# drwangxian/viterbi_spl

Hardware: AMD Instinct MI355X
Metric: Viterbi Mframes/s at S=361 T=30k; achieved HBM GB/s vs peak (higher is better)
Workload: dtype f32

## Files before the change

### viterbi_spl_amd/csrc/banded.hip

```cpp
#include "device_common.hpp"

namespace vit {

template <int W, int NWT, bool DW, bool DBG, int NXT, typename ET>
__global__ void __launch_bounds__((NWT + (DW ? 3 : 2)) * 64) banded_forward_kernel(FwdArgs a) {
    extern __shared__ __align__(16) unsigned char smem[];
    constexpr int NP = NWT * 64;
    constexpr int EPL = NWT;
    const int S = a.S, SP = a.SP, T = a.T, SD = a.SD;
    constexpr int DC = NP + 16;
    float* dls = reinterpret_cast<float*>(smem);
    float* dl = dls + 4;
    float* Pv = dls + 4 * DC;
    float* Sv = Pv + NP + 1;
    float* Dv = Sv + NP + 1;
    VI* tot = reinterpret_cast<VI*>(Dv + kMaxDenseRows);

    const int tid = threadIdx.x;
    const int lane = tid & 63;
    const int wv = __builtin_amdgcn_readfirstlane(tid >> 6);
    const int song = blockIdx.x;
    const int Tb = song_length(a.lengths, song, T);
    const ET* __restrict__ E = reinterpret_cast<const ET*>(a.logE) + (size_t)song * T * S;
    float* __restrict__ hist = a.hist + (size_t)song * T * SD;
// ... 85 lines not shown
        unsigned long long v;
        asm volatile("s_memtime %0\n\ts_waitcnt lgkmcnt(0)" : "=s"(v)::"memory");
        return v;
    };
    auto frame = [&](const int t, float& e_slot) {
        float m = -INFINITY;
        const bool prof = (dbg & 256) != 0;
        const unsigned long long s0 = prof ? stamp() : 0ull;
        if (is_target) {
            float m0 = -INFINITY, m1 = -INFINITY, m2 = -INFINITY, m3 = -INFINITY;
            float xd[NXL > 0 ? NXL : 1];
#pragma unroll
            for (int k = 0; k < NXL; ++k) xd[k] = (!GEN || k < nx) ? dl[xcol[k]] : -INFINITY;
            if (!(dbg & 1)) {
                const f32x4* __restrict__ win = reinterpret_cast<const f32x4*>(dl + (lo & 3) * DC + (lo & ~3));
#pragma unroll
                for (int w = 0; w + 7 < W; w += 8) {
                    const f32x4 da = win[w / 4], db = win[w / 4 + 1];
                    const f32x2 c0_ = f32x2{da.x, da.y} + f32x2{aw[w + 0], aw[w + 1]};
                    const f32x2 c1_ = f32x2{da.z, da.w} + f32x2{aw[w + 2], aw[w + 3]};
                    const f32x2 c2_ = f32x2{db.x, db.y} + f32x2{aw[w + 4], aw[w + 5]};
                    const f32x2 c3_ = f32x2{db.z, db.w} + f32x2{aw[w + 6], aw[w + 7]};
                    m0 = fmaxf(fmaxf(m0, c0_.x), c0_.y);
                    m1 = fmaxf(fmaxf(m1, c1_.x), c1_.y);
                    m2 = fmaxf(fmaxf(m2, c2_.x), c2_.y);
                    m3 = fmaxf(fmaxf(m3, c3_.x), c3_.y);
                }
            }
#pragma unroll
            for (int k = 0; k < NXL; ++k) m1 = fmaxf(m1, xd[k] + xa[k]);
            m = fmaxf(fmaxf(m0, m1), fmaxf(m2, m3));
        } else if (!(dbg & 2)) {
            float d[EPL];
#pragma unroll
            for (int e = 0; e < EPL; ++e) d[e] = dl[i0 + e];
            if (role == 0) {
                float p[EPL];
                float run = -INFINITY;
#pragma unroll
                for (int e = 0; e < EPL; ++e) {
                    run = fmaxf(run, smask[e] ? -INFINITY : d[e]);
                    p[e] = run;
                }
                const float inc = wave_scan_max(run);
                const float ex = wave_shift_up(inc, -INFINITY);
#pragma unroll
                for (int e = 0; e < EPL; ++e) Pv[i0 + e + 1] = fmaxf(ex, p[e]);
                if (lane == 63 && !(dbg & 8)) hist[(size_t)(t - 1) * SD + S] = inc;
            } else {
                if (role == 1) {
                    float p[EPL];
                    float run = -INFINITY;
#pragma unroll
                    for (int e = EPL - 1; e >= 0; --e) {
                        run = fmaxf(run, smask[e] ? -INFINITY : d[e]);
                        p[e] = run;
                    }
                    const float ex = wave_shift_up(wave_scan_max(run), -INFINITY);
#pragma unroll
                    for (int e = 0; e < EPL; ++e) Sv[i0 + e] = fmaxf(ex, p[e]);
                }
                if (GEN && role == kDenseRole) {
#pragma unroll
                    for (int dr = 0; dr < kMaxDenseRows; ++dr) {
                        if (dr < nd) {
                            float dm = -INFINITY;
#pragma unroll
                            for (int e = 0; e < EPL; ++e) dm = fmaxf(dm, d[e] + dA[dr][e]);
                            dm = wave_max_all(dm);
                            if (lane == 0) Dv[dr] = dm;
                        }
                    }
                }
            }
        }
        const unsigned long long s1 = prof ? stamp() : 0ull;
        __syncthreads();
        const unsigned long long s2 = prof ? stamp() : 0ull;

        if (is_target && !(dbg & 4)) {
            m = fmaxf(m, fmaxf(Pv[lo], Sv[lo + W]) + cj);
            if (GEN) {
                const float dres = Dv[kind >= 0 ? kind : 0];
                if (kind >= 0) m = dres;
            }
            {
                const float dn = tvalid ? m + e_slot : -INFINITY;
#pragma unroll
                for (int c = 0; c < 4; ++c) dl[c * DC + j - c] = dn;
                if (!(dbg & 8)) {
                    float* __restrict__ hrow = hist + (size_t)t * SD;
                    const int tn = t + 2 < Tb ? t + 2 : Tb - 1;
                    const ET* __restrict__ erow = E + (size_t)tn * S;
                    hrow[jst] = dn;
                    e_slot = load_e<ET>(erow + jld);
                }
            }
        }
        const unsigned long long s3 = prof ? stamp() : 0ull;
        __syncthreads();
        if (prof) {
            const unsigned long long s4 = stamp();
            ph0 += s1 - s0; ph1 += s2 - s1; ph2 += s3 - s2; ph3 += s4 - s3;
        }
    };
    const unsigned long long clk0 = (dbg & 48) ? __builtin_amdgcn_s_memtime() : 0ull;
    const unsigned long long rt0 = (dbg & 48) ? __builtin_amdgcn_s_memrealtime() : 0ull;
    int t = 1;
    for (; t + 1 < Tb; t += 2) {
        frame(t, e_a);
        frame(t + 1, e_b);
    }
    if (t < Tb) frame(t, e_a);

    terminal_argmax(is_target ? dl[j] : -INFINITY, j, tvalid, tot, NWT + (DW ? 3 : 2), a.last_state, a.loglik, song);
    if ((dbg & 256) && lane == 0 && Tb > 1) {
        float* o = a.fmax + (size_t)song * 64 + 4 * wv;
        const float n = (float)(Tb - 1);
        o[0] = (float)ph0 / n; o[1] = (float)ph1 / n; o[2] = (float)ph2 / n; o[3] = (float)ph3 / n;
    }
    if ((dbg & 48) && tid == 0) {
        const unsigned long long d = (dbg & 16) ? __builtin_amdgcn_s_memtime() - clk0 : __builtin_amdgcn_s_memrealtime() - rt0;
        a.fmax[(size_t)song * 64 + 63] = (float)d / (float)(Tb > 1 ? Tb - 1 : 1);
    }
}

#include "banded_floor.inc"

constexpr int split_waitcnt(int vm, int lgkm) { return (vm & 15) | ((vm >> 4) << 14) | (7 << 4) | (lgkm << 8); }
constexpr int kNoVmWait = 63;
constexpr int split_reads_behind(int NQ, int g) { return (NQ + 1) - 2 * (g + 1); }
template <int... K, typename F>
__device__ __forceinline__ void split_frames(std::integer_sequence<int, K...>, F&& f) { (f(std::integral_constant<int, K>{}), ...); }
template <int NXT, int PF, typename ET, bool WPR = false, bool XQ = false, int WF = 32>
__global__ void __launch_bounds__(64 * (kSplitFullWaves + kSplitHalfWaves)) banded_floor_split_forward_kernel(FwdArgs a) {
    extern __shared__ __align__(16) unsigned char smem[];
    constexpr int W = 32;
    static_assert(WF == W || (WF % 4 == 1 && WF >= 9 && WF < W && NXT == 1), "a trimmed window: whole quads and one float, one extra column");
    constexpr int NWF = kSplitFullWaves, NW = kSplitFullWaves + kSplitHalfWaves;
    using L = FloorSplitLds;
    constexpr int DC = L::DC, BUF = L::BUF;
    float* dls = reinterpret_cast<float*>(smem) + L::dls;
    float* fmg = dls + L::fmg;
    VI* tot = reinterpret_cast<VI*>(dls + L::tot);
    const int S = a.S, SP = a.SP, T = a.T, SD = a.SD;
    constexpr bool GEN = NXT < 0;
    constexpr int NXL = GEN ? kMaxExtras : NXT;
    const int nx = GEN ? a.n_extras : NXT;

    const int tid = threadIdx.x;
    const int lane = tid & 63;
    const int wv = __builtin_amdgcn_readfirstlane(tid >> 6);
    const bool half = wv >= NWF;
    const int hh = half ? lane >> 5 : 0;
    const int song = blockIdx.x;
    const int Tb = song_length(a.lengths, song, T);
    const ET* __restrict__ E = reinterpret_cast<const ET*>(a.logE) + (size_t)song * T * S;
    float* __restrict__ hist = a.hist + (size_t)song * T * SD;

    const int j = half ? 64 * NWF + 32 * (wv - NWF) + (lane & 31) : tid;
    const bool tvalid = j < S;
    const bool own = tvalid && hh == 0;
    const int jc = tvalid ? j : 0;
    const int jld = tvalid ? j : S - 1;
    const bool is_fm = j == S;
    const unsigned hoff = tvalid ? (unsigned)(SD + j) : (is_fm ? (unsigned)S : (unsigned)(SD + S + 1));
    const unsigned hoffb = 4u * hoff, eoffb = (unsigned)(sizeof(ET) * jld);
    const int lo = reinterpret_cast<const int32_t*>(a.image + a.off_lo)[jc];
    int xcol[NXL > 0 ? NXL : 1];
    bool is_x = false;
#pragma unroll
    for (int k = 0; k < NXL; ++k) {
        xcol[k] = k < nx ? a.extras[k] : 0;
        is_x |= (k < nx && j == xcol[k]);
    }
    const int sh = a.win_shift;
    const int lov = (tvalid ? lo : 0) + sh;
    const float* rp = dls + 4 + (lov & 3) * DC + (lov & ~3) + 16 * hh;
    float* fmp = fmg + fm_slot((XQ && is_x) ? (lane | 1) : lane);
    static_assert(!XQ || NXT == 1, "the extra column leaves M by address only where the launcher proved its quad idle");

    for (int k = tid; k < L::reset; k += NW * 64) dls[k] = -INFINITY;
    __syncthreads();

#ifdef VIT_TIMING_HOOKS
    const bool probe = (a.debug & 48) != 0;
    constexpr bool wprobe = WPR;
    WaveProbe wp_;
#else
    constexpr bool probe = false;
#endif
    unsigned long long clk0 = 0ull, rt0 = 0ull;

    auto body = [&](auto role, auto resets) {
        constexpr bool HALF = decltype(role)::value, RESETS = decltype(resets)::value;
        constexpr int WL = HALF ? W / 2 : WF;
        constexpr bool TRIM = WL % 4 != 0;
        const float cj = own ? reinterpret_cast<const float*>(a.image + a.off_rowc)[jc] : -INFINITY;
        float aw[WL];
        float xa[NXL > 0 ? NXL : 1];
        {
            const float* __restrict__ tab = reinterpret_cast<const float*>(a.image + a.off_tabA);
            const float* __restrict__ xaT = reinterpret_cast<const float*>(a.image + a.off_extraA);
#pragma unroll
            for (int w = 0; w < WL; ++w) aw[w] = tvalid ? tab[(size_t)(w + (HALF ? 16 * hh : 0)) * SP + jc] : -INFINITY;
#pragma unroll
            for (int k = 0; k < NXL; ++k)
                xa[k] = (tvalid && k < nx && (!HALF || hh == 1)) ? xaT[(size_t)k * SP + jc] : -INFINITY;
        }
        float* wp = dls + 4 + sh + j + (HALF ? hh * split_upper_off(DC) : 0);
        int xo[NXL > 0 ? NXL : 1];
#pragma unroll
        for (int k = 0; k < NXL; ++k) {
            xo[k] = 4 + sh + xcol[k];
            asm volatile("" : "+v"(xo[k]));
        }

        auto produce = [&](const float dn, const int WB, const int G, const int Z) {
#pragma unroll
            for (int c = 0; c < (HALF ? 2 : 4); ++c) wp[WB * BUF + floor_copy_off(DC, c)] = dn;
            fm_publish(fmp + G * kFmGroupFloats, (!XQ && NXL > 0 && is_x) ? -INFINITY : dn);
            if constexpr (RESETS) fmg[Z * kFmGroupFloats + lane] = -INFINITY;
        };

        {
            const float d0 = tvalid ? reinterpret_cast<const float*>(a.image + a.off_logpi)[j] + load_e<ET>(E + j) : -INFINITY;
            if (own) hist[j] = d0;
            produce(d0, 0, 0, 1);
        }
        float er[PF];
#pragma unroll
        for (int k = 0; k < PF; ++k) er[k] = load_e<ET>(E + (size_t)(1 + k < Tb ? 1 + k : Tb - 1) * S + jld);
#pragma unroll
        for (int w = 0; w < WL; ++w) asm volatile("" ::"v"(aw[w]));
#pragma unroll
        for (int k = 0; k < NXL; ++k) asm volatile("" ::"v"(xa[k]));
        asm volatile("" ::"v"(cj));
        __syncthreads();

        const unsigned rowH = 4u * (unsigned)SD, rowE = (unsigned)sizeof(ET) * (unsigned)S;
        float* hb = hist;
        const ET* eb = E;
        unsigned elim = 0;
        auto round_bases = [&](const int t) {
            const int r = t + PF < Tb ? t + PF : Tb - 1;
            const int ahead = Tb - 1 - r < PF ? Tb - 1 - r : PF;
            hb = hist + (size_t)(t - 1) * SD;
            eb = E + (size_t)r * S;
            elim = (unsigned)ahead * rowE;
        };
        auto frame = [&](float& e_slot, auto uc) {
            constexpr int u = decltype(uc)::value;
            const int RB = u & 1, WB = RB ^ 1;
            const int GR = u % kFmGroups, GW = (u + 1) % kFmGroups, GZ = (u + 2) % kFmGroups;
            const f32x4* __restrict__ win = reinterpret_cast<const f32x4*>(rp + RB * BUF);
            float xd[NXL > 0 ? NXL : 1];
            f32x4 fq;
            [[maybe_unused]] float m0, m1 = -INFINITY, m2 = -INFINITY, m3 = -INFINITY;
#pragma unroll
            for (int k = 0; k < NXL; ++k) xd[k] = dls[xo[k] + RB * BUF];
            fq = reinterpret_cast<const f32x4*>(fmg + GR * kFmGroupFloats)[0];
            asm volatile("" ::: "memory");
            f32x4 dw[WL / 4];
#pragma unroll
            for (int q = 0; q < WL / 4; ++q) dw[q] = win[q];
            [[maybe_unused]] float ds = 0.f;
            if constexpr (TRIM) ds = (rp + RB * BUF)[WL - 1];
            __builtin_amdgcn_sched_barrier(0);
            if constexpr (TRIM) {
                static_assert(split_reads_behind(WL / 4, 0) == WL / 4 + 1 - 2, "behind the first pair: every other window read of the burst");
                __builtin_amdgcn_s_waitcnt(split_waitcnt(kNoVmWait, split_reads_behind(WL / 4, 0)));
                asm volatile("" : "+v"(fq), "+v"(dw[0]), "+v"(dw[1]));
            }
            const float M = fmaxf(fmaxf(fq.x, fq.y), fmaxf(fq.z, fq.w));
            m0 = M + cj;
            asm volatile("" ::"v"(m0));
            __builtin_amdgcn_sched_barrier(0);
            float mx;
            constexpr int vmw = PF - 1 + u;
            static_assert(vmw <= 2 * (PF - 1) && 2 * (PF - 1) < kNoVmWait, "vmcnt bound: one store and one load per frame, 6-bit field");
            if constexpr (TRIM) {
                constexpr int NQ = WL / 4, TQ = NQ % 2 ? 1 : 2, NPB = (NQ - TQ) / 2;
                static_assert(NXL == 1 && NQ >= 3 && 2 * NPB + TQ == NQ && 4 * NQ + 1 == WL, "pairs of quads, then the tail: one or two quads and one float");
                static_assert(split_reads_behind(NQ, 0) <= 15, "lgkmcnt is a four-bit field");
                static_assert(split_reads_behind(NQ, NPB - 1) == TQ + 1, "behind the last pair stand the tail's reads -- TQ quads and the float -- and nothing else");
                static_assert(split_reads_behind(NQ, NPB) + 2 == TQ + 1 && TQ <= 2, "the tail's wait, lgkmcnt(0), leaves no window read out");
                float mb = xd[0] + xa[0];
                asm volatile("" ::"v"(mb));
                split_frames(std::make_integer_sequence<int, NPB>{}, [&](auto gc) {
                    constexpr int w = 8 * decltype(gc)::value;
                    f32x4 da = dw[w / 4], db = dw[w / 4 + 1];
                    if constexpr (decltype(gc)::value >= 1) {
                        constexpr int behind = split_reads_behind(NQ, decltype(gc)::value);
                        static_assert(behind >= TQ + 1 && behind + 2 == split_reads_behind(NQ, decltype(gc)::value - 1), "two reads fewer than the pair before");
                        __builtin_amdgcn_s_waitcnt(split_waitcnt(kNoVmWait, behind));
                        asm volatile("" : "+v"(da), "+v"(db));
                    }
                    f32x2 c0_ = f32x2{da.x, da.y} + f32x2{aw[w + 0], aw[w + 1]};
                    f32x2 c1_ = f32x2{da.z, da.w} + f32x2{aw[w + 2], aw[w + 3]};
                    f32x2 c2_ = f32x2{db.x, db.y} + f32x2{aw[w + 4], aw[w + 5]};
                    f32x2 c3_ = f32x2{db.z, db.w} + f32x2{aw[w + 6], aw[w + 7]};
                    asm volatile("" : "+v"(c0_), "+v"(c1_), "+v"(c2_), "+v"(c3_));
                    m0 = fmaxf(fmaxf(m0, c0_.x), c0_.y);
                    mb = fmaxf(fmaxf(mb, c1_.x), c1_.y);
                    m0 = fmaxf(fmaxf(m0, c2_.x), c2_.y);
                    mb = fmaxf(fmaxf(mb, c3_.x), c3_.y);
                });
                {
                    constexpr int w = 8 * NPB;
                    f32x4 da = dw[w / 4], db = dw[NQ - 1];
                    __builtin_amdgcn_s_waitcnt(split_waitcnt(vmw, 0));
                    if constexpr (TQ == 2) asm volatile("" : "+v"(da), "+v"(db), "+v"(ds)); else asm volatile("" : "+v"(da), "+v"(ds));
                    f32x2 c0_ = f32x2{da.x, da.y} + f32x2{aw[w + 0], aw[w + 1]};
                    f32x2 c1_ = f32x2{da.z, da.w} + f32x2{aw[w + 2], aw[w + 3]};
                    float cs = ds + aw[WL - 1];
                    if constexpr (TQ == 2) {
                        f32x2 c2_ = f32x2{db.x, db.y} + f32x2{aw[w + 4], aw[w + 5]};
                        f32x2 c3_ = f32x2{db.z, db.w} + f32x2{aw[w + 6], aw[w + 7]};
                        asm volatile("" : "+v"(c0_), "+v"(c1_), "+v"(c2_), "+v"(c3_), "+v"(cs));
                        m0 = fmaxf(fmaxf(m0, c0_.x), c0_.y);
                        mb = fmaxf(fmaxf(mb, c1_.x), c1_.y);
                        m0 = fmaxf(fmaxf(m0, c2_.x), c2_.y);
                        mb = fmaxf(fmaxf(mb, c3_.x), c3_.y);
                    } else {
                        asm volatile("" : "+v"(c0_), "+v"(c1_), "+v"(cs));
                        m0 = fmaxf(fmaxf(m0, c0_.x), c0_.y);
                        mb = fmaxf(fmaxf(mb, c1_.x), c1_.y);
                    }
                    mx = fmaxf(fmaxf(m0, mb), cs);
                }
            } else {
                split_frames(std::make_integer_sequence<int, WL / 8>{}, [&](auto gc) {
                    constexpr int w = 8 * decltype(gc)::value;
                    constexpr bool last = w + 8 == WL;
                    constexpr bool pairw = w + 16 >= WL && w >= 8;
                    f32x4 da = dw[w / 4], db = dw[w / 4 + 1];
                    if constexpr (pairw) {
                        __builtin_amdgcn_s_waitcnt(split_waitcnt(last ? vmw : kNoVmWait, last ? 0 : 2));
                        asm volatile("" : "+v"(da), "+v"(db));
                    }
                    f32x2 c0_ = f32x2{da.x, da.y} + f32x2{aw[w + 0], aw[w + 1]};
                    f32x2 c1_ = f32x2{da.z, da.w} + f32x2{aw[w + 2], aw[w + 3]};
                    f32x2 c2_ = f32x2{db.x, db.y} + f32x2{aw[w + 4], aw[w + 5]};
                    f32x2 c3_ = f32x2{db.z, db.w} + f32x2{aw[w + 6], aw[w + 7]};
                    asm volatile("" : "+v"(c0_), "+v"(c1_), "+v"(c2_), "+v"(c3_));
                    m0 = fmaxf(fmaxf(m0, c0_.x), c0_.y);
                    m1 = fmaxf(fmaxf(m1, c1_.x), c1_.y);
                    m2 = fmaxf(fmaxf(m2, c2_.x), c2_.y);
                    m3 = fmaxf(fmaxf(m3, c3_.x), c3_.y);
                });
#pragma unroll
                for (int k = 0; k < NXL; ++k) m1 = fmaxf(m1, xd[k] + xa[k]);
                mx = fmaxf(fmaxf(m0, m1), fmaxf(m2, m3));
            }
            if constexpr (HALF) mx = max_other_half(mx);
            const float dn = mx + e_slot;
#ifdef VIT_TIMING_HOOKS
            if constexpr (wprobe) wp_.before_publish(dn);
#endif
            const float sv = (HALF && is_fm) ? M : dn;
            const unsigned eso = (unsigned)u * rowE < elim ? (unsigned)u * rowE : elim;
            produce(dn, WB, GW, GZ);
            asm volatile("" ::: "memory");
            row_store_f32(hb, hoffb, sv, (unsigned)u * rowH);
            e_slot = row_load_e<ET>(eb, eoffb, eso);
#ifdef VIT_TIMING_HOOKS
            if constexpr (wprobe) wp_.barrier(); else
#endif
            __syncthreads();
        };
#ifdef VIT_TIMING_HOOKS
        if constexpr (wprobe) wp_.start();
#endif
        clk0 = probe ? __builtin_amdgcn_s_memtime() : 0ull;
        rt0 = probe ? __builtin_amdgcn_s_memrealtime() : 0ull;
        if constexpr (HALF) __builtin_amdgcn_s_setprio(1);
        int t = 1;
        for (; t + PF - 1 < Tb; t += PF) {
            round_bases(t);
            split_frames(std::make_integer_sequence<int, PF>{}, [&](auto k) { frame(er[k], k); });
        }
        round_bases(t);
        split_frames(std::make_integer_sequence<int, PF - 1>{}, [&](auto k) {
            if (t + k < Tb) frame(er[k], k);
        });
    };
    static_assert(PF % 2 == 0 && PF % kFmGroups == 0, "the unrolled frames must cycle through whole buffer and slot-group rounds");
    if (!half) body(std::false_type{}, std::false_type{});
    else if (wv == NW - 1) body(std::true_type{}, std::true_type{});
    else body(std::true_type{}, std::false_type{});

    const int fb = (Tb - 1) & 1;
    terminal_argmax(own ? dls[4 + sh + fb * BUF + j] : -INFINITY, j, own, tot, NW, a.last_state, a.loglik, song);
    if (probe && tid == 0) {
        const unsigned long long d = (a.debug & 16) ? __builtin_amdgcn_s_memtime() - clk0 : __builtin_amdgcn_s_memrealtime() - rt0;
        a.fmax[(size_t)song * 64 + 63] = (float)d / (float)(Tb > 1 ? Tb - 1 : 1);
    }
#ifdef VIT_TIMING_HOOKS
    if constexpr (wprobe) wp_.finish(a.fmax + (size_t)song * 64, wv, lane, Tb - 1);
#endif
}

template <int NPW>
struct FloorPairLds {
    static constexpr int NP = NPW * 128;
    static constexpr int DC = NP + 16;
    static constexpr int BUF = 4 * DC;
    static constexpr int NWM = (NPW + 3) / 4 * 4;
    static constexpr int dls = 0;
    static constexpr int wm = dls + 2 * BUF;
    static constexpr int reset = wm + 2 * NWM;
    static constexpr int dump = reset;
    static constexpr int tot = dump + 64 + NWM;
    static constexpr int end = tot + 16 * (int)(sizeof(VI) / sizeof(float));
    static_assert(sizeof(float) * end <= kLdsBytes, "one workgroup's LDS");
    static constexpr size_t bytes() { return sizeof(float) * end; }
};

template <int W, int NPW, int NXT, int PF, typename ET>
__global__ void __launch_bounds__(NPW * 64) banded_floor_pair_forward_kernel(FwdArgs a) {
    extern __shared__ __align__(16) unsigned char smem[];
    using L = FloorPairLds<NPW>;
    constexpr int DC = L::DC, BUF = L::BUF, NWM = L::NWM;
    float* dls = reinterpret_cast<float*>(smem) + L::dls;
    float* wm = dls + L::wm;
    float* dump = dls + L::dump;
    VI* tot = reinterpret_cast<VI*>(dls + L::tot);
    const int S = a.S, SP = a.SP, T = a.T, SD = a.SD;
    constexpr bool GEN = NXT < 0;
    constexpr int NXL = GEN ? kMaxExtras : NXT;
    const int nx = GEN ? a.n_extras : NXT;

    const int tid = threadIdx.x;
    const int lane = tid & 63;
    const int wv = __builtin_amdgcn_readfirstlane(tid >> 6);
    const int song = blockIdx.x;
    const int Tb = song_length(a.lengths, song, T);
    const ET* __restrict__ E = reinterpret_cast<const ET*>(a.logE) + (size_t)song * T * S;
    float* __restrict__ hist = a.hist + (size_t)song * T * SD;

    const int j0 = 2 * tid, j1 = 2 * tid + 1;
    const bool v0 = j0 < S, v1 = j1 < S;
    const int jc0 = v0 ? j0 : 0, jc1 = v1 ? j1 : jc0;
    const int jl0 = v0 ? j0 : S - 1, jl1 = v1 ? j1 : S - 1;
    const unsigned hoff0 = v0 ? (unsigned)(SD + j0) : (j0 == S ? (unsigned)S : (unsigned)(SD + S + 1));
    const unsigned hoff1 = v1 ? (unsigned)(SD + j1) : (j1 == S ? (unsigned)S : (unsigned)(SD + S + 1));
    const bool fm0 = j0 == S, fm1 = j1 == S;
    const int lo2 = v0 ? reinterpret_cast<const int32_t*>(a.image + a.off_lo2)[jc0 >> 1] : 0;
    const float* __restrict__ rc = reinterpret_cast<const float*>(a.image + a.off_rowc);
    f32x2 cj = f32x2{v0 ? rc[jc0] : -INFINITY, v1 ? rc[jc1] : -INFINITY};
    float aw0[W], aw1[W];
    f32x2 xa[NXL > 0 ? NXL : 1];
    int xcol[NXL > 0 ? NXL : 1];
    bool x0 = false, x1 = false;
    {
        const float* __restrict__ tab = reinterpret_cast<const float*>(a.image + a.off_tabP);
        const float* __restrict__ xaT = reinterpret_cast<const float*>(a.image + a.off_extraA);
#pragma unroll
        for (int w = 0; w < W; ++w) {
            aw0[w] = v0 ? tab[(size_t)w * SP + jc0] : -INFINITY;
            aw1[w] = v1 ? tab[(size_t)w * SP + jc1] : -INFINITY;
        }
#pragma unroll
        for (int k = 0; k < NXL; ++k) {
            xcol[k] = k < nx ? a.extras[k] : 0;
            xa[k] = f32x2{(v0 && k < nx) ? xaT[(size_t)k * SP + jc0] : -INFINITY, (v1 && k < nx) ? xaT[(size_t)k * SP + jc1] : -INFINITY};
            x0 |= (k < nx && j0 == xcol[k]);
            x1 |= (k < nx && j1 == xcol[k]);
        }
    }
    const int sh = a.win_shift2;
    const int lov = lo2 + sh;
    const float* rp = dls + 4 + (lov & 3) * DC + (lov & ~3);
    float* wp = dls + 4 + sh + j0;
    float* wmp = lane == 63 ? wm + wv : dump + lane;

    for (int k = tid; k < L::reset; k += NPW * 64) dls[k] = -INFINITY;
    __syncthreads();

    auto produce = [&](const f32x2 dn, const int WB) {
#pragma unroll
        for (int c = 0; c < 4; ++c) {
            wp[WB * BUF + c * DC - c] = dn.x;
            wp[WB * BUF + c * DC - c + 1] = dn.y;
        }
        const float inc = wave_scan_max(fmaxf((NXL > 0 && x0) ? -INFINITY : dn.x, (NXL > 0 && x1) ? -INFINITY : dn.y));
        wmp[WB * NWM] = inc;
    };

    {
        const float* __restrict__ lpi = reinterpret_cast<const float*>(a.image + a.off_logpi);
        f32x2 d0 = f32x2{-INFINITY, -INFINITY};
        if (v0) { d0.x = lpi[j0] + load_e<ET>(E + j0); hist[j0] = d0.x; }
        if (v1) { d0.y = lpi[j1] + load_e<ET>(E + j1); hist[j1] = d0.y; }
        produce(d0, 0);
    }
    f32x2 er[PF];
#pragma unroll
    for (int k = 0; k < PF; ++k) {
        const ET* __restrict__ row = E + (size_t)(1 + k < Tb ? 1 + k : Tb - 1) * S;
        er[k] = f32x2{load_e<ET>(row + jl0), load_e<ET>(row + jl1)};
    }
#pragma unroll
    for (int w = 0; w < W; ++w) asm volatile("" ::"v"(aw0[w]), "v"(aw1[w]));
#pragma unroll
    for (int k = 0; k < NXL; ++k) asm volatile("" ::"v"(xa[k]));
    asm volatile("" ::"v"(cj));
    __syncthreads();
// ... 228 lines not shown
```

### viterbi_spl_amd/csrc/banded_floor.inc

```
__device__ __forceinline__ __amdgpu_buffer_rsrc_t row_rsrc(const void* row) {
    return __builtin_amdgcn_make_buffer_rsrc(const_cast<void*>(row), (short)0, -1, 0x00020000);
}
__device__ __forceinline__ void row_store_f32(float* row, unsigned off, float v, unsigned soff = 0) {
    __builtin_amdgcn_raw_buffer_store_b32(__float_as_uint(v), row_rsrc(row), off, soff, 0);
}
template <typename ET>
__device__ __forceinline__ float row_load_e(const ET* row, unsigned off, unsigned soff = 0);
template <>
__device__ __forceinline__ float row_load_e<float>(const float* row, unsigned off, unsigned soff) {
    return __uint_as_float(__builtin_amdgcn_raw_buffer_load_b32(row_rsrc(row), off, soff, 0));
}
template <>
__device__ __forceinline__ float row_load_e<__half>(const __half* row, unsigned off, unsigned soff) {
    return __half2float(__ushort_as_half(__builtin_amdgcn_raw_buffer_load_b16(row_rsrc(row), off, soff, 0)));
}

inline constexpr int kFmGroups = 4;
inline constexpr int kFmGroupFloats = 64;
inline constexpr int kFmSlots = 4;
__device__ __forceinline__ int fm_slot(int lane) { return 4 * (lane & 3) + ((lane >> 2) & 3); }
__device__ __forceinline__ void fm_publish(float* slot, float v) {
    v = fmaxf(v, __int_as_float(__builtin_amdgcn_update_dpp(0, __float_as_int(v), 0xb1, 0xf, 0xf, false)));
    v = fmaxf(v, __int_as_float(__builtin_amdgcn_update_dpp(0, __float_as_int(v), 0x4e, 0xf, 0xf, false)));
    __hip_atomic_fetch_max(slot, v, __ATOMIC_RELAXED, __HIP_MEMORY_SCOPE_WORKGROUP);
}

#ifdef VIT_TIMING_HOOKS
struct WaveProbe {
    unsigned long long t_rel = 0, t_pub = 0, work = 0, wait = 0;
    __device__ __forceinline__ void start() { t_rel = __builtin_amdgcn_s_memtime(); }
    __device__ __forceinline__ void before_publish(float dn) {
        __builtin_amdgcn_sched_barrier(0);
        asm volatile("" ::"v"(dn));
        t_pub = __builtin_amdgcn_s_memtime();
        __builtin_amdgcn_sched_barrier(0);
    }
    __device__ __forceinline__ void barrier() {
        unsigned long long t_in, t_out;
        asm volatile("s_waitcnt lgkmcnt(0)\n\ts_memtime %0\n\ts_barrier\n\ts_memtime %1\n\ts_waitcnt lgkmcnt(0)"
                     : "=&s"(t_in), "=&s"(t_out) : "s"(t_pub) : "memory");
        work += t_pub - t_rel;
        wait += t_out - t_in;
        t_rel = t_out;
    }
    __device__ __forceinline__ void finish(float* scratch, int wv, int lane, int frames) const {
        if (lane != 0) return;
        const float n = (float)(frames > 0 ? frames : 1);
        scratch[4 * wv + 0] = (float)__builtin_amdgcn_s_getreg((1 << 11) | (4 << 6) | 4);
        scratch[4 * wv + 1] = (float)work / n;
        scratch[4 * wv + 2] = (float)wait / n;
        scratch[4 * wv + 3] = n;
    }
};
#endif

template <int W, int NWT, WgVariant V = WgVariant::Plain>
struct FloorLds {
    static constexpr int NP = NWT * 64;
    static constexpr int DC = NP + 16;
    static constexpr int BUF = 4 * DC;
    static constexpr int WR = (W == 128 && NWT > 8) ? (V != WgVariant::Plain ? 88 : 96) : W;
    static constexpr int dls = 0;
    static constexpr int fmg = dls + 2 * BUF;
    static constexpr int reset = fmg + kFmGroups * kFmGroupFloats;
    static constexpr int tot = reset;
    static constexpr int awl = tot + 16 * (int)(sizeof(VI) / sizeof(float));
    static constexpr int end = awl + (W - WR) / 4 * 4 * NP;
    static_assert(sizeof(float) * end <= kLdsBytes, "one workgroup's LDS");
    static constexpr size_t bytes() { return sizeof(float) * end; }
};
constexpr int floor_copy_off(int DC, int c) { return c * DC - c; }
constexpr int split_upper_off(int DC) { return floor_copy_off(DC, 2); }
inline constexpr int kSplitFullWaves = 4, kSplitHalfWaves = 4;
inline constexpr int kSplitStates = 64 * kSplitFullWaves + 32 * kSplitHalfWaves;
using FloorSplitLds = FloorLds<32, kSplitStates / 64>;

template <int W, int NWT, int NXT, int PF, typename ET, WgVariant V = WgVariant::Plain, bool WPR = false>
__global__ void __launch_bounds__(NWT * 64) banded_floor_forward_kernel(FwdArgs a) {
    static_assert(!WPR || V == WgVariant::Plain, "the per-wave probe exists for the plain kernel only");
    using L = FloorLds<W, NWT, V>;
    constexpr bool PK = V == WgVariant::Packed, CK = V == WgVariant::Ckpt, PC = V == WgVariant::PackedCkpt;
    constexpr bool PKx = PK || PC;
    constexpr bool CKx = CK || PC;
    extern __shared__ __align__(16) unsigned char smem[];
    constexpr int NP = L::NP, DC = L::DC, BUF = L::BUF, WR = L::WR;
    float* dls = reinterpret_cast<float*>(smem) + L::dls;
    float* fmg = dls + L::fmg;
    VI* tot = reinterpret_cast<VI*>(dls + L::tot);
    f32x4* awl = reinterpret_cast<f32x4*>(dls + L::awl);
    const int S = a.S, SP = a.SP, T = a.T, SD = a.SD;
    constexpr bool GEN = NXT < 0;
    constexpr int NXL = GEN ? kMaxExtras : NXT;
    const int nx = GEN ? a.n_extras : NXT;

    const int tid = threadIdx.x;
    const int lane = tid & 63;
    const int wv = __builtin_amdgcn_readfirstlane(tid >> 6);
    constexpr int kPast = 1, kRowBias = 1;
#define VIT_WG_CURSOR 1
#include "wg_cursor.inc"
#define VIT_WG_CURSOR 2
#include "wg_cursor.inc"

    const int j = tid;
    const bool tvalid = j < S;
    const int jc = tvalid ? j : 0;
    const int jld = tvalid ? j : S - 1;
    const unsigned hoff = tvalid ? (unsigned)(SD + j) : ((j == S && !(CKx && ck_every > 0)) ? (unsigned)S : (unsigned)(SD + S + 1));
    const bool is_fm = j == S;
    const unsigned hoffb = 4u * hoff, eoffb = (unsigned)(sizeof(ET) * jld);
    const int lo = reinterpret_cast<const int32_t*>(a.image + a.off_lo)[jc];
    const float cj = tvalid ? reinterpret_cast<const float*>(a.image + a.off_rowc)[jc] : -INFINITY;
    float aw[WR];
    float xa[NXL > 0 ? NXL : 1];
    int xcol[NXL > 0 ? NXL : 1];
    bool is_x = false;
    {
        const float* __restrict__ tab = reinterpret_cast<const float*>(a.image + a.off_tabA);
        const float* __restrict__ xaT = reinterpret_cast<const float*>(a.image + a.off_extraA);
#pragma unroll
        for (int w = 0; w < WR; ++w) aw[w] = tvalid ? tab[(size_t)w * SP + jc] : -INFINITY;
#pragma unroll
        for (int q = 0; q < (W - WR) / 4; ++q) {
            f32x4 wv4;
            wv4.x = tvalid ? tab[(size_t)(WR + 4 * q + 0) * SP + jc] : -INFINITY;
            wv4.y = tvalid ? tab[(size_t)(WR + 4 * q + 1) * SP + jc] : -INFINITY;
            wv4.z = tvalid ? tab[(size_t)(WR + 4 * q + 2) * SP + jc] : -INFINITY;
            wv4.w = tvalid ? tab[(size_t)(WR + 4 * q + 3) * SP + jc] : -INFINITY;
            awl[q * NP + j] = wv4;
        }
#pragma unroll
        for (int k = 0; k < NXL; ++k) {
            xcol[k] = k < nx ? a.extras[k] : 0;
            xa[k] = (tvalid && k < nx) ? xaT[(size_t)k * SP + jc] : -INFINITY;
            is_x |= (k < nx && j == xcol[k]);
        }
    }
    const int sh = a.win_shift;
    const int lov = (tvalid ? lo : 0) + sh;
    const float* rp = dls + 4 + (lov & 3) * DC + (lov & ~3);
    float* wp = dls + 4 + sh + j;
    float* fmp = fmg + fm_slot(lane);

    for (int k = tid; k < L::reset; k += NWT * 64) dls[k] = -INFINITY;
    __syncthreads();

    auto produce = [&](const float dn, const int WB, const int G, const int Z) {
#pragma unroll
        for (int c = 0; c < 4; ++c) wp[WB * BUF + floor_copy_off(DC, c)] = dn;
        fm_publish(fmp + G * kFmGroupFloats, (NXL > 0 && is_x) ? -INFINITY : dn);
        int w = wv;
        asm volatile("" : "+s"(w));
        if (w == NWT - 1) fmg[Z * kFmGroupFloats + lane] = -INFINITY;
    };

    for (;;) {
        int jf = j;
        if constexpr (PKx) asm volatile("" : "+v"(jf));
        const bool tvf = PKx ? jf < S : tvalid;
        const int jldf = PKx ? (tvf ? jf : S - 1) : jld;
        if constexpr (CKx) {
            float d0 = -INFINITY;
            if (t0 > 0) {
                if (tvf) d0 = PC ? pc_init[jf] : a.init_rows[(size_t)song * a.init_stride + jf];
            } else if (tvf) {
                d0 = reinterpret_cast<const float*>(a.image + a.off_logpi)[jf] + load_e<ET>(E + jf);
                hist[(size_t)(ck_every > 0 ? ck_scratch : 0) * SD + jf] = d0;
            }
            produce(d0, 0, 0, 1);
        } else {
            const float d0 = tvf ? reinterpret_cast<const float*>(a.image + a.off_logpi)[jf] + load_e<ET>(E + jf) : -INFINITY;
            if (tvf) hist[jf] = d0;
            produce(d0, 0, 0, 1);
        }
        float er[PF];
#pragma unroll
        for (int k = 0; k < PF; ++k) er[k] = load_e<ET>(E + (size_t)((CKx ? t1 : 1) + k < Tb ? (CKx ? t1 : 1) + k : Tb - 1) * S + jldf);
#pragma unroll
        for (int w = 0; w < WR; ++w) asm volatile("" ::"v"(aw[w]));
#pragma unroll
        for (int k = 0; k < NXL; ++k) asm volatile("" ::"v"(xa[k]));
        asm volatile("" ::"v"(cj));
        __syncthreads();

        static_assert(PF % 2 == 0 && PF % kFmGroups == 0, "the unrolled frames must cycle through whole buffer and slot-group rounds");
#ifdef VIT_TIMING_HOOKS
        constexpr bool wprobe = WPR;
        WaveProbe wp_;
#endif
        auto frame = [&](const int t, float& e_slot, const int u) {
            const int RB = u & 1, WB = RB ^ 1;
            const int GR = u % kFmGroups, GW = (u + 1) % kFmGroups, GZ = (u + 2) % kFmGroups;
            const f32x4* __restrict__ win = reinterpret_cast<const f32x4*>(rp + RB * BUF);
            float xd[NXL > 0 ? NXL : 1];
            f32x4 fq[kFmSlots / 4];
            auto small_reads = [&]() {
#pragma unroll
                for (int k = 0; k < NXL; ++k) xd[k] = dls[4 + sh + RB * BUF + xcol[k]];
#pragma unroll
                for (int q = 0; q < kFmSlots / 4; ++q) fq[q] = reinterpret_cast<const f32x4*>(fmg + GR * kFmGroupFloats)[q];
            };
            float m0 = -INFINITY, m1 = -INFINITY, m2 = -INFINITY, m3 = -INFINITY;
            float M = -INFINITY;
            small_reads();
            asm volatile("" ::: "memory");
#pragma unroll
            for (int w0 = 0; w0 < W; w0 += 32) {
            if ((W > 64 || (W == 64 && NWT > 8)) && w0 > 0) asm volatile("" : "+v"(m0), "+v"(m1), "+v"(m2), "+v"(m3)::"memory");
            f32x4 dw[8];
#ifdef VIT_ABL_READS
#pragma unroll
            for (int q = 0; q < 8; ++q)
                if (w0 + 4 * q < W) { if (q < VIT_ABL_READS) dw[q] = win[w0 / 4 + q]; else dw[q] = dw[q % VIT_ABL_READS]; }
#else
#pragma unroll
            for (int q = 0; q < 8; ++q)
                if (w0 + 4 * q < W) dw[q] = win[w0 / 4 + q];
#endif
            if (w0 == 0) {
                __builtin_amdgcn_sched_barrier(0);
                M = fmaxf(fmaxf(fq[0].x, fq[0].y), fmaxf(fq[0].z, fq[0].w));
#pragma unroll
                for (int q = 1; q < kFmSlots / 4; ++q) M = fmaxf(fmaxf(fmaxf(M, fq[q].x), fq[q].y), fmaxf(fq[q].z, fq[q].w));
                m0 = M + cj;
                __builtin_amdgcn_sched_barrier(0);
            }
#pragma unroll
            for (int w = w0; w + 7 < W && w < w0 + 32; w += 8) {
// ... 155 lines not shown
```

### viterbi_spl_amd/csrc/device_common.hpp

```cpp
#pragma once
#include <hip/hip_fp16.h>
#include <hip/hip_runtime.h>

#include <cstddef>
#include <cstdint>
#include <type_traits>

#include "kernels.hpp"

namespace vit {

inline constexpr int kBig = 0x7fffffff;
inline constexpr size_t kLdsBytes = 160 * 1024;

typedef float f32x2 __attribute__((ext_vector_type(2)));
typedef float f32x4 __attribute__((ext_vector_type(4)));
typedef float f32x4_u __attribute__((ext_vector_type(4), aligned(4)));
typedef float f32x2_u __attribute__((ext_vector_type(2), aligned(4)));
typedef int i32x4_u __attribute__((ext_vector_type(4), aligned(4)));
typedef _Float16 f16x2_u __attribute__((ext_vector_type(2), aligned(2)));
typedef _Float16 f16x4_u __attribute__((ext_vector_type(4), aligned(2)));

__device__ __forceinline__ int song_length(const int64_t* lengths, int song, int T) {
    if (!lengths) return T;
    long long v = lengths[song];
    v = v < 1 ? 1 : v;
    return v > T ? T : (int)v;
}
__device__ __forceinline__ int clamp_med3(int x, int hi) {
    int r;
    asm("v_med3_i32 %0, %1, 0, %2" : "=v"(r) : "v"(x), "s"(hi));
    return r;
}

template <typename ET>
__device__ __forceinline__ float load_e(const ET* p);
template <>
__device__ __forceinline__ float load_e<float>(const float* p) { return *p; }
template <>
__device__ __forceinline__ float load_e<__half>(const __half* p) { return __half2float(*p); }

__device__ __forceinline__ float wave_scan_max(float x) {
    asm volatile(
        "s_nop 1\n\t"
        "v_max_f32_dpp %0, %0, %0 row_shr:1 row_mask:0xf bank_mask:0xf\n\t"
        "s_nop 1\n\t"
        "v_max_f32_dpp %0, %0, %0 row_shr:2 row_mask:0xf bank_mask:0xf\n\t"
        "s_nop 1\n\t"
        "v_max_f32_dpp %0, %0, %0 row_shr:4 row_mask:0xf bank_mask:0xf\n\t"
        "s_nop 1\n\t"
        "v_max_f32_dpp %0, %0, %0 row_shr:8 row_mask:0xf bank_mask:0xf\n\t"
        "s_nop 1\n\t"
        "v_max_f32_dpp %0, %0, %0 row_bcast:15 row_mask:0xa bank_mask:0xf\n\t"
        "s_nop 1\n\t"
        "v_max_f32_dpp %0, %0, %0 row_bcast:31 row_mask:0xc bank_mask:0xf\n\t"
        "s_nop 1"
        : "+v"(x));
    return x;
}
__device__ __forceinline__ float wave_max_all(float x) {
    return __int_as_float(__builtin_amdgcn_readlane(__float_as_int(wave_scan_max(x)), 63));
}
__device__ __forceinline__ float max_other_half(float x) {
    const auto r = __builtin_amdgcn_permlane32_swap(__float_as_uint(x), __float_as_uint(x), false, false);
    return fmaxf(__uint_as_float(r[0]), __uint_as_float(r[1]));
}
__device__ __forceinline__ float wave_shift_up(float x, float fill) {
    return __int_as_float(__builtin_amdgcn_update_dpp(__float_as_int(fill), __float_as_int(x), 0x138, 0xf, 0xf, false));
}
__device__ __forceinline__ float wave_shift_down(float x, float fill) {
    return __int_as_float(__builtin_amdgcn_update_dpp(__float_as_int(fill), __float_as_int(x), 0x130, 0xf, 0xf, false));
}
__device__ __forceinline__ float dpp_shr1(float x) {
    return __int_as_float(__builtin_amdgcn_update_dpp(0, __float_as_int(x), 0x138, 0xf, 0xf, true));
}
__device__ __forceinline__ float dpp_shl1(float x) {
    return __int_as_float(__builtin_amdgcn_update_dpp(0, __float_as_int(x), 0x130, 0xf, 0xf, true));
}

struct VI {
    float v;
    int i;
};

__device__ __forceinline__ VI vi_identity() { return VI{-INFINITY, kBig}; }
__device__ __forceinline__ VI op_fwd(VI earlier, VI later) { return later.v > earlier.v ? later : earlier; }
__device__ __forceinline__ VI op_rev(VI acc, VI next) { return next.v >= acc.v ? next : acc; }

template <int CTRL, int ROW_MASK>
__device__ __forceinline__ VI dpp_fetch(VI x) {
    VI r;
    r.v = __int_as_float(__builtin_amdgcn_update_dpp(__float_as_int(-INFINITY), __float_as_int(x.v), CTRL,
                                                     ROW_MASK, 0xf, false));
    r.i = __builtin_amdgcn_update_dpp(kBig, x.i, CTRL, ROW_MASK, 0xf, false);
    return r;
}

template <bool REV>
__device__ __forceinline__ VI wave_scan(VI x) {
#define VIT_SCAN_STEP(CTRL, MASK)                        \
    {                                                    \
        VI s = dpp_fetch<CTRL, MASK>(x);                 \
        x = REV ? op_rev(s, x) : op_fwd(s, x);           \
    }
    VIT_SCAN_STEP(0x111, 0xf)
    VIT_SCAN_STEP(0x112, 0xf)
    VIT_SCAN_STEP(0x114, 0xf)
    VIT_SCAN_STEP(0x118, 0xf)
    VIT_SCAN_STEP(0x142, 0xa)
    VIT_SCAN_STEP(0x143, 0xc)
#undef VIT_SCAN_STEP
    return x;
}

__device__ __forceinline__ void terminal_argmax(float dj, int j, bool valid, VI* tot, int nw, int32_t* last_state,
                                                float* loglik, int song) {
    VI x{valid ? dj : -INFINITY, valid ? j : kBig};
    x = wave_scan<false>(x);
    if ((threadIdx.x & 63) == 63) tot[threadIdx.x >> 6] = x;
    __syncthreads();
    if (threadIdx.x == 0) {
        VI acc = vi_identity();
        for (int b = 0; b < nw; ++b) acc = op_fwd(acc, tot[b]);
        if (acc.i == kBig) acc.i = 0;
        last_state[song] = acc.i;
        if (loglik) loglik[song] = acc.v;
    }
}

__device__ __forceinline__ void terminal_argmax_w(float dj, int j, bool valid, VI* tot, int nw, int wave, int lane, int32_t* last_state,
                                                  float* loglik, int song) {
    VI x{valid ? dj : -INFINITY, valid ? j : kBig};
    x = wave_scan<false>(x);
    if (lane == 63) tot[wave] = x;
    __syncthreads();
    if (wave == 0 && lane == 0) {
        VI acc = vi_identity();
        for (int b = 0; b < nw; ++b) acc = op_fwd(acc, tot[b]);
        if (acc.i == kBig) acc.i = 0;
        last_state[song] = acc.i;
        if (loglik) loglik[song] = acc.v;
    }
}

}
```

### viterbi_spl_amd/csrc/floor_lds_check.hip

```cpp
#include <cstdio>
#include <cstdlib>
#include <vector>

#include "device_common.hpp"

namespace vit {
#include "banded_floor.inc"
}
using namespace vit;

static int failures = 0;
#define CHECK(cond, ...)                                                     \
    do {                                                                     \
        if (!(cond)) {                                                       \
            if (++failures <= 20) { std::printf("FAIL %s: ", #cond); std::printf(__VA_ARGS__); std::printf("\n"); } \
        }                                                                    \
    } while (0)

static bool write2_encodable(int stride) { return stride >= 0 && stride <= 255; }
static bool write2st64_encodable(int stride) { return stride >= 0 && stride % 64 == 0 && stride / 64 <= 255; }

struct Segment {
    std::vector<int> owner;
    explicit Segment(int n) : owner((size_t)n, -1) {}
    void claim(int pos, int tag, const char* what, int W, int NWT) {
        CHECK(pos >= 0 && pos < (int)owner.size(), "%s at %d outside the segment of %zu floats (W %d, NWT %d)", what, pos, owner.size(), W, NWT);
        if (pos < 0 || pos >= (int)owner.size()) return;
        CHECK(owner[(size_t)pos] == -1 || owner[(size_t)pos] == tag, "%s at %d: tag %d collides with %d (W %d, NWT %d)", what, pos, tag, owner[(size_t)pos], W, NWT);
        owner[(size_t)pos] = tag;
    }
};

template <typename L, int W>
static void replay(const char* name, int NWT, bool split) {
    constexpr int NP = L::NP, DC = L::DC, BUF = L::BUF;
    static_assert(DC % 4 == 0, "a copy starts on a 16-byte boundary");
    CHECK(L::fmg == 2 * BUF && L::reset == L::fmg + kFmGroups * kFmGroupFloats && L::end >= L::awl, "%s: carving order", name);
    for (int sh = 0; sh < 4; ++sh) {
        Segment seg(L::end);
        for (int b = 0; b < 2; ++b)
            for (int c = 0; c < 4; ++c)
                for (int j = 0; j < NP; ++j) {
                    const int pos = L::dls + 4 + sh + j + b * BUF + floor_copy_off(DC, c);
                    CHECK(pos >= L::dls + b * BUF + c * DC && pos < L::dls + b * BUF + (c + 1) * DC, "%s: write of delta[%d] leaves copy %d (sh %d)", name, j, c, sh);
                    seg.claim(pos, 16 * b + c, "delta copy", W, NWT);
                }
        for (int g = 0; g < kFmGroups; ++g)
            for (int l = 0; l < kFmGroupFloats; ++l) seg.claim(L::fmg + g * kFmGroupFloats + l, 64 + g, "slot group", W, NWT);
        for (int k = L::tot; k < L::end; ++k) seg.claim(k, 128, "terminal scratch / LDS-resident weights", W, NWT);
        for (int S = 1; S < NP; ++S) {
            const int lo_max = S - W > 0 ? S - W : 0;
            for (int lo = 0; lo <= lo_max; ++lo) {
                const int lov = lo + sh, r = lov & 3;
                for (int hh = 0; hh < (split ? 2 : 1); ++hh) {
                    const int WL = split ? W / 2 : W;
                    const int rp = L::dls + 4 + r * DC + (lov & ~3) + (split ? 16 * hh : 0);
                    for (int b = 0; b < 2; ++b) {
                        const int first = rp + b * BUF, last = first + WL - 1;
                        CHECK(first % 4 == 0, "%s: window read at %d not 16-byte aligned (lo %d, sh %d)", name, first, lo, sh);
                        CHECK(first >= L::dls + b * BUF + r * DC && last < L::dls + b * BUF + (r + 1) * DC,
                              "%s: window [%d, %d] leaves copy %d of buffer %d (S %d, lo %d, sh %d)", name, first, last, r, b, S, lo, sh);
                        const int i0 = first - (L::dls + b * BUF + r * DC) - 4 - sh + r;
                        CHECK(i0 == lo + (split ? 16 * hh : 0), "%s: window starts at delta[%d], not delta[%d] (sh %d)", name, i0, lo + 16 * hh, sh);
                    }
                }
            }
        }
    }
    if (split) {
        for (int sh = 0; sh < 4; ++sh)
            for (int wv = kSplitFullWaves; wv < kSplitFullWaves + kSplitHalfWaves; ++wv)
                for (int lane = 0; lane < 64; ++lane) {
                    const int hh = lane >> 5, j = 64 * kSplitFullWaves + 32 * (wv - kSplitFullWaves) + (lane & 31);
                    CHECK(j >= 64 * kSplitFullWaves && j < kSplitStates, "split target %d", j);
                    const int wp = L::dls + 4 + sh + j + hh * split_upper_off(DC);
                    for (int c = 0; c < 2; ++c) {
                        const int r = 2 * hh + c, pos = wp + floor_copy_off(DC, c);
                        CHECK(pos == L::dls + r * DC + 4 + sh + j - r, "split lane %d of wave %d: copy %d written at %d (sh %d)", lane, wv, r, pos, sh);
                    }
                }
    }
    const int stride = DC - 1;
    bool residues[4] = {false, false, false, false};
    for (int c = 0; c < 4; ++c) residues[(c * stride) & 3] = true;
    CHECK(residues[0] && residues[1] && residues[2] && residues[3], "%s: the four copies must cover the four alignments", name);
    bool any64 = false;
    for (int c0 = 0; c0 < 4; ++c0)
        for (int c1 = c0 + 1; c1 < 4; ++c1) any64 |= write2st64_encodable((c1 - c0) * stride);
    CHECK(!any64, "%s: an st64 pair would mean two copies with the same alignment", name);
    const bool plain = write2_encodable(stride);
    CHECK(plain == (NP + 15 <= 255), "%s: plain pair iff a copy fits 255 dwords", name);
    std::printf("%-28s NP %4d DC %4d bytes %6zu  copy stride %4d dwords: ds_write2_b32 %s, ds_write2st64_b32 no\n", name, NP, DC, L::bytes(),
                stride, plain ? "pairs (0,1) and (2,3)" : "no");
}

template <int W, int NWT>
static void replay_pair() {
    char name[64];
    std::snprintf(name, sizeof name, "FloorLds<%d, %d>", W, NWT);
    replay<FloorLds<W, NWT, WgVariant::Plain>, W>(name, NWT, false);
    if constexpr (W == 128 && NWT > 8) {
        std::snprintf(name, sizeof name, "FloorLds<%d, %d, Packed>", W, NWT);
        replay<FloorLds<W, NWT, WgVariant::Packed>, W>(name, NWT, false);
    }
}
template <int W>
static void replay_width() {
    replay_pair<W, 2>();
    replay_pair<W, 4>();
    replay_pair<W, 6>();
    replay_pair<W, 8>();
    replay_pair<W, 12>();
}

int main() {
    static_assert(sizeof(kBandedWidths) / sizeof(int) == 6, "one call per instantiated window width");
    replay_width<16>();
    replay_width<32>();
    replay_width<64>();
    replay_width<84>();
    replay_width<96>();
    replay_width<128>();
    replay<FloorSplitLds, 32>("FloorSplitLds (split kernel)", kSplitStates / 64, true);
    static_assert(2 * FloorSplitLds::bytes() <= kLdsBytes && 2 * FloorLds<32, 6>::bytes() <= kLdsBytes, "two workgroups share a CU's LDS");
    if (failures) { std::printf("%d check(s) failed\n", failures); return 1; }
    std::printf("floor LDS layouts: all checks passed\n");
    return 0;
}
```

Before: 494.3.

## Remap split-kernel half lanes to xor-8 partners and route extra column via M slot

In the split Viterbi kernel, the two halves of each half-wave are now paired as lane and lane^8 instead of 32 lanes apart. Their cross-half max then uses a single DPP row_ror:8 instead of a permlane32 swap, and the mapping is meant to cut LDS bank conflicts on the ds_read_b128 window reads. When XQ is set, the extra column's value is carried in the fourth slot of the frame-max vector, which drops the separate per-frame LDS read of the extra column. Host-side checks are added to validate the new lane map, slot map and read-cycle counts, and out-of-range targets now clamp their window base to S-W.

```diff
diff --git a/viterbi_spl_amd/csrc/banded.hip b/viterbi_spl_amd/csrc/banded.hip
--- a/viterbi_spl_amd/csrc/banded.hip
+++ b/viterbi_spl_amd/csrc/banded.hip
@@ -261,13 +261,13 @@
     const int lane = tid & 63;
     const int wv = __builtin_amdgcn_readfirstlane(tid >> 6);
     const bool half = wv >= NWF;
-    const int hh = half ? lane >> 5 : 0;
+    const int hh = half ? split_half_of(lane) : 0;
     const int song = blockIdx.x;
     const int Tb = song_length(a.lengths, song, T);
     const ET* __restrict__ E = reinterpret_cast<const ET*>(a.logE) + (size_t)song * T * S;
     float* __restrict__ hist = a.hist + (size_t)song * T * SD;
 
-    const int j = half ? 64 * NWF + 32 * (wv - NWF) + (lane & 31) : tid;
+    const int j = half ? 64 * NWF + 32 * (wv - NWF) + split_half_target(lane) : tid;
     const bool tvalid = j < S;
     const bool own = tvalid && hh == 0;
     const int jc = tvalid ? j : 0;
@@ -284,9 +284,10 @@
         is_x |= (k < nx && j == xcol[k]);
     }
     const int sh = a.win_shift;
-    const int lov = (tvalid ? lo : 0) + sh;
+    const int lov = (tvalid ? lo : S - W) + sh;
     const float* rp = dls + 4 + (lov & 3) * DC + (lov & ~3) + 16 * hh;
-    float* fmp = fmg + fm_slot((XQ && is_x) ? (lane | 1) : lane);
+    constexpr bool XS = XQ;
+    float* fmp = fmg + (XS ? split_fm_slot(lane, is_x) : fm_slot(lane));
     static_assert(!XQ || NXT == 1, "the extra column leaves M by address only where the launcher proved its quad idle");
 
     for (int k = tid; k < L::reset; k += NW * 64) dls[k] = -INFINITY;
@@ -318,11 +319,13 @@
                 xa[k] = (tvalid && k < nx && (!HALF || hh == 1)) ? xaT[(size_t)k * SP + jc] : -INFINITY;
         }
         float* wp = dls + 4 + sh + j + (HALF ? hh * split_upper_off(DC) : 0);
-        int xo[NXL > 0 ? NXL : 1];
-#pragma unroll
-        for (int k = 0; k < NXL; ++k) {
-            xo[k] = 4 + sh + xcol[k];
-            asm volatile("" : "+v"(xo[k]));
+        [[maybe_unused]] int xo[NXL > 0 ? NXL : 1];
+        if constexpr (!XS) {
+#pragma unroll
+            for (int k = 0; k < NXL; ++k) {
+                xo[k] = 4 + sh + xcol[k];
+                asm volatile("" : "+v"(xo[k]));
+            }
         }
 
         auto produce = [&](const float dn, const int WB, const int G, const int Z) {
@@ -366,8 +369,10 @@
             float xd[NXL > 0 ? NXL : 1];
             f32x4 fq;
             [[maybe_unused]] float m0, m1 = -INFINITY, m2 = -INFINITY, m3 = -INFINITY;
-#pragma unroll
-            for (int k = 0; k < NXL; ++k) xd[k] = dls[xo[k] + RB * BUF];
+            if constexpr (!XS) {
+#pragma unroll
+                for (int k = 0; k < NXL; ++k) xd[k] = dls[xo[k] + RB * BUF];
+            }
             fq = reinterpret_cast<const f32x4*>(fmg + GR * kFmGroupFloats)[0];
             asm volatile("" ::: "memory");
             f32x4 dw[WL / 4];
@@ -381,7 +386,8 @@
                 __builtin_amdgcn_s_waitcnt(split_waitcnt(kNoVmWait, split_reads_behind(WL / 4, 0)));
                 asm volatile("" : "+v"(fq), "+v"(dw[0]), "+v"(dw[1]));
             }
-            const float M = fmaxf(fmaxf(fq.x, fq.y), fmaxf(fq.z, fq.w));
+            const float M = XS ? fmaxf(fmaxf(fq.x, fq.y), fq.z) : fmaxf(fmaxf(fq.x, fq.y), fmaxf(fq.z, fq.w));
+            if constexpr (XS) xd[0] = fq.w;
             m0 = M + cj;
             asm volatile("" ::"v"(m0));
             __builtin_amdgcn_sched_barrier(0);
@@ -462,7 +468,7 @@
                 for (int k = 0; k < NXL; ++k) m1 = fmaxf(m1, xd[k] + xa[k]);
                 mx = fmaxf(fmaxf(m0, m1), fmaxf(m2, m3));
             }
-            if constexpr (HALF) mx = max_other_half(mx);
+            if constexpr (HALF) mx = max_lane_xor8(mx);
             const float dn = mx + e_slot;
 #ifdef VIT_TIMING_HOOKS
             if constexpr (wprobe) wp_.before_publish(dn);
diff --git a/viterbi_spl_amd/csrc/banded_floor.inc b/viterbi_spl_amd/csrc/banded_floor.inc
--- a/viterbi_spl_amd/csrc/banded_floor.inc
+++ b/viterbi_spl_amd/csrc/banded_floor.inc
@@ -74,6 +74,10 @@
 inline constexpr int kSplitFullWaves = 4, kSplitHalfWaves = 4;
 inline constexpr int kSplitStates = 64 * kSplitFullWaves + 32 * kSplitHalfWaves;
 using FloorSplitLds = FloorLds<32, kSplitStates / 64>;
+constexpr int split_half_of(int lane) { return (lane >> 3) & 1; }
+constexpr int split_half_target(int lane) { return ((lane >> 4) << 3) | (lane & 7); }
+inline constexpr int kSplitXSlot = 3;
+constexpr int split_fm_slot(int lane, bool is_x) { return 4 * (lane & 3) + (is_x ? kSplitXSlot : (lane >> 2) % 3); }
 
 template <int W, int NWT, int NXT, int PF, typename ET, WgVariant V = WgVariant::Plain, bool WPR = false>
 __global__ void __launch_bounds__(NWT * 64) banded_floor_forward_kernel(FwdArgs a) {
diff --git a/viterbi_spl_amd/csrc/device_common.hpp b/viterbi_spl_amd/csrc/device_common.hpp
--- a/viterbi_spl_amd/csrc/device_common.hpp
+++ b/viterbi_spl_amd/csrc/device_common.hpp
@@ -64,6 +64,10 @@
 __device__ __forceinline__ float max_other_half(float x) {
     const auto r = __builtin_amdgcn_permlane32_swap(__float_as_uint(x), __float_as_uint(x), false, false);
     return fmaxf(__uint_as_float(r[0]), __uint_as_float(r[1]));
+}
+inline constexpr int kDppRowRor8 = 0x128;
+__device__ __forceinline__ float max_lane_xor8(float x) {
+    return fmaxf(x, __int_as_float(__builtin_amdgcn_update_dpp(0, __float_as_int(x), kDppRowRor8, 0xf, 0xf, false)));
 }
 __device__ __forceinline__ float wave_shift_up(float x, float fill) {
     return __int_as_float(__builtin_amdgcn_update_dpp(__float_as_int(fill), __float_as_int(x), 0x138, 0xf, 0xf, false));
diff --git a/viterbi_spl_amd/csrc/floor_lds_check.hip b/viterbi_spl_amd/csrc/floor_lds_check.hip
--- a/viterbi_spl_amd/csrc/floor_lds_check.hip
+++ b/viterbi_spl_amd/csrc/floor_lds_check.hip
@@ -71,7 +71,7 @@
         for (int sh = 0; sh < 4; ++sh)
             for (int wv = kSplitFullWaves; wv < kSplitFullWaves + kSplitHalfWaves; ++wv)
                 for (int lane = 0; lane < 64; ++lane) {
-                    const int hh = lane >> 5, j = 64 * kSplitFullWaves + 32 * (wv - kSplitFullWaves) + (lane & 31);
+                    const int hh = split_half_of(lane), j = 64 * kSplitFullWaves + 32 * (wv - kSplitFullWaves) + split_half_target(lane);
                     CHECK(j >= 64 * kSplitFullWaves && j < kSplitStates, "split target %d", j);
                     const int wp = L::dls + 4 + sh + j + hh * split_upper_off(DC);
                     for (int c = 0; c < 2; ++c) {
@@ -94,6 +94,121 @@
                 stride, plain ? "pairs (0,1) and (2,3)" : "no");
 }
 
+static int old_half_of(int lane) { return lane >> 5; }
+static int old_half_target(int lane) { return lane & 31; }
+static void replay_lane_map() {
+    int next = 0;
+    for (int lane = 0; lane < 64; ++lane) {
+        const int hh = split_half_of(lane), k = split_half_target(lane), p = lane ^ 8;
+        CHECK(hh == 0 || hh == 1, "lane %d: half %d", lane, hh);
+        CHECK(k >= 0 && k < 32, "lane %d: target %d", lane, k);
+        CHECK(split_half_target(p) == k && split_half_of(p) == 1 - hh, "lane %d: partner %d holds target %d half %d", lane, p, split_half_target(p), split_half_of(p));
+        CHECK((lane >> 4) == (p >> 4), "lane %d: partner %d in another DPP row", lane, p);
+        CHECK((k & 3) == (lane & 3), "lane %d: target %d sits elsewhere in its quad", lane, k);
+        if (hh == 0) { CHECK(k == next, "lower lane %d takes target %d, not %d", lane, k, next); ++next; }
+    }
+    CHECK(next == 32, "%d lower lanes", next);
+    std::printf("split lane map: partner l ^ 8 (row_ror:8), 32 lower lanes in ascending target order: ok\n");
+}
+
+static int read_b128_cycles(const int* addr ) {
+    static const int groups[4][16] = {{0, 1, 2, 3, 12, 13, 14, 15, 20, 21, 22, 23, 24, 25, 26, 27},
+                                      {4, 5, 6, 7, 8, 9, 10, 11, 16, 17, 18, 19, 28, 29, 30, 31},
+                                      {32, 33, 34, 35, 44, 45, 46, 47, 52, 53, 54, 55, 56, 57, 58, 59},
+                                      {36, 37, 38, 39, 40, 41, 42, 43, 48, 49, 50, 51, 60, 61, 62, 63}};
+    int cycles = 0;
+    for (int g = 0; g < 4; ++g) {
+        int worst = 1;
+        for (int bank = 0; bank < 64; bank += 4) {
+            int seen[16], n = 0;
+            for (int i = 0; i < 16; ++i) {
+                const int a = addr[groups[g][i]];
+                if (a % 64 != bank) continue;
+                bool dup = false;
+                for (int q = 0; q < n; ++q) dup |= seen[q] == a;
+                if (!dup) seen[n++] = a;
+            }
+            if (n > worst) worst = n;
+        }
+        cycles += worst;
+    }
+    return cycles;
+}
+template <typename HF, typename TF>
+static int half_wave_read_cycles(int S, int off, int sh, int hw, HF half_of, TF target_of) {
+    using L = FloorSplitLds;
+    constexpr int W = 32;
+    int cycles = 0;
+    for (int q = 0; q < W / 2 / 4; ++q) {
+        int addr[64];
+        for (int lane = 0; lane < 64; ++lane) {
+            const int j = 64 * kSplitFullWaves + 32 * hw + target_of(lane);
+            int lo = j - off;
+            lo = lo < 0 ? 0 : (lo > S - W ? S - W : lo);
+            const int lov = (j < S ? lo : S - W) + sh;
+            addr[lane] = L::dls + 4 + (lov & 3) * L::DC + (lov & ~3) + 16 * half_of(lane) + 4 * q;
+        }
+        cycles += read_b128_cycles(addr);
+    }
+    return cycles;
+}
+static void replay_read_cycles(int S, int off) {
+    for (int sh = 0; sh < 4; ++sh) {
+        int was[kSplitHalfWaves], now[kSplitHalfWaves];
+        for (int hw = 0; hw < kSplitHalfWaves; ++hw) {
+            was[hw] = half_wave_read_cycles(S, off, sh, hw, old_half_of, old_half_target);
+            now[hw] = half_wave_read_cycles(S, off, sh, hw, split_half_of, split_half_target);
+            if (sh == off % 4) CHECK(now[hw] <= was[hw], "S %d sh %d half wave %d: %d LDS cycles for its window reads, %d with the halves 32 lanes apart", S, sh, hw, now[hw], was[hw]);
+        }
+        std::printf("split window reads S %d off %d sh %d%s: ds_read_b128 cycles per half wave, halves 32 lanes apart %d / %d / %d / %d, partner l ^ 8 %d / %d / %d / %d\n",
+                    S, off, sh, sh == off % 4 ? " (the plan's)" : "", was[0], was[1], was[2], was[3], now[0], now[1], now[2], now[3]);
+    }
+}
+
+static void replay_slot_map() {
+    int cases = 0;
+    for (int S = 64 * kSplitFullWaves + 1; S < kSplitStates; S += 4) {
+        const int x = S - 1;
+        CHECK(x % 4 == 0, "x %d", x);
+        bool x_reached = false;
+        for (int wv = 0; wv < kSplitFullWaves + kSplitHalfWaves; ++wv) {
+            bool quad_in_m[16] = {};
+            for (int lane = 0; lane < 64; ++lane) {
+                const bool half = wv >= kSplitFullWaves;
+                const int j = half ? 64 * kSplitFullWaves + 32 * (wv - kSplitFullWaves) + split_half_target(lane) : 64 * wv + lane;
+                const int slot = split_fm_slot(lane, j == x);
+                CHECK(slot >= 0 && slot < 16, "slot %d", slot);
+                bool quad_has_x = false;
+                for (int m = 0; m < 4; ++m) {
+                    const int lm = (lane & ~3) | m;
+                    const int jm = half ? 64 * kSplitFullWaves + 32 * (wv - kSplitFullWaves) + split_half_target(lm) : 64 * wv + lm;
+                    quad_has_x |= jm == x;
+                    if (quad_has_x && jm != x) CHECK(jm >= S, "S %d: state %d shares a quad with x and is live", S, jm);
+                }
+                if (slot < kSplitXSlot) {
+                    CHECK(!quad_has_x, "S %d wave %d lane %d: a quad that holds x adds into M slot %d", S, wv, lane, slot);
+                    quad_in_m[lane >> 2] = true;
+                }
+                if (slot == kSplitXSlot) {
+                    CHECK(j == x, "S %d wave %d lane %d (state %d) adds into the extra column's slot", S, wv, lane, j);
+                    x_reached = true;
+                }
+            }
+            for (int q = 0; q < 16; ++q) {
+                bool has_x = false;
+                for (int m = 0; m < 4; ++m) {
+                    const int lm = 4 * q + m;
+                    has_x |= (wv >= kSplitFullWaves ? 64 * kSplitFullWaves + 32 * (wv - kSplitFullWaves) + split_half_target(lm) : 64 * wv + lm) == x;
+                }
+                CHECK(quad_in_m[q] != has_x, "S %d wave %d quad %d: %s", S, wv, q, has_x ? "holds x and reaches M" : "reaches none of slots 0 .. 2");
+            }
+        }
+        CHECK(x_reached, "S %d: no lane adds x into slot %d", S, kSplitXSlot);
+        ++cases;
+    }
+    std::printf("split slot map: every quad without x reaches one of slots 0 .. 2, x reaches slot %d alone: ok (%d state counts)\n", kSplitXSlot, cases);
+}
+
 template <int W, int NWT>
 static void replay_pair() {
     char name[64];
@@ -122,6 +237,10 @@
     replay_width<96>();
     replay_width<128>();
     replay<FloorSplitLds, 32>("FloorSplitLds (split kernel)", kSplitStates / 64, true);
+    replay_lane_map();
+    replay_slot_map();
+    replay_read_cycles(361, 15);
+    replay_read_cycles(321, 13);
     static_assert(2 * FloorSplitLds::bytes() <= kLdsBytes && 2 * FloorLds<32, 6>::bytes() <= kLdsBytes, "two workgroups share a CU's LDS");
     if (failures) { std::printf("%d check(s) failed\n", failures); return 1; }
     std::printf("floor LDS layouts: all checks passed\n");
```

Result: faster. 506.1, median of 6 (+2.4%).
